# monahand1023/imageclust

Measured on AMD Instinct MI355X. Metric: images/sec (embed+Ward), higher is better.
Workload: dtype bf16; 1 GPU; the metric's size (configs[2]'s N=100000) on 1 GPU: 100000 synthetic 224x224x3 images (structured, seed 20250217; 100000 on this rank), ResNet50-v1 bf16 batch=256 -> 2048-d pooled E -> Ward min=5 max=50 (merge loop on GPU0) -> cluster ids on host; n_images_total=100000, embed_dim=2048, weights=synthetic seed 1, device=AMD Radeon Graphics (gfx950:sramecc+:xnack-)

## Files before the change

### imageclust_amd/csrc/ward.hip

```cpp
#pragma clang fp contract(off)

#include "icl_common.h"
#include "mfma_tile.h"
#include "ward_value.h"
typedef float f32x4 __attribute__((ext_vector_type(4)));

#include <algorithm>
#include <cmath>
#include <cstring>
#include <type_traits>

int icl_dist_mfma_launch(icl_ctx *ctx, const float *d_E, int64_t n, int d, float *d_out, const int64_t *d_rowoff, int64_t ld);
int icl_dist_center_launch(icl_ctx *ctx, const float *d_E, int64_t n, int d, int K, double *d_colsum, float *d_Ec, float *d_nrm, hipStream_t strm);
size_t icl_dist_colsum_doubles(int d);
int icl_dist_bound_launch(icl_ctx *ctx, const float *d_Ec, const float *d_nrm, const void *d_zero, int64_t n, int K, float ceps, float gam, float *d_out,
                          const int64_t *d_rowoff, int64_t tr_lo, int64_t tr_hi, hipStream_t strm);

bool icl_dist_i8_usable(int64_t n, int d);
size_t icl_dist_i8_pq_bytes(int64_t n, int d);
int icl_dist_bound_i8_launch(icl_ctx *ctx, const float *d_Ec, const float *d_nrm, int64_t n, int d, int K, float gam, void *d_pq, float *d_l1, int32_t *d_ex,
                             float *d_out, const int64_t *d_rowoff, hipStream_t strm, unsigned int *d_rowub);

typedef float f2 __attribute__((ext_vector_type(2)));

// ... 8 lines not shown
#define WB_R 128
#endif
#define WB_RL ((WB_R + 63) / 64)
#ifndef WB_NSP_LB
#define WB_NSP_LB 128
#endif
#define WB_NSP_X 64
#ifndef WB_SCAN_U
#define WB_SCAN_U 4
#endif
#ifndef WB_RM
#define WB_RM 2
#endif
__device__ __forceinline__ int wb_poll(const int32_t *p) { return __hip_atomic_load(p, __ATOMIC_RELAXED, __HIP_MEMORY_SCOPE_AGENT); }
__device__ __forceinline__ void wb_acquire() { __builtin_amdgcn_fence(__ATOMIC_ACQUIRE, "agent"); }
#define WB_NN_BOUND (-2)
#ifndef WB_LAZY_TOP
#define WB_LAZY_TOP 1
#endif
#define WB_PA_CAP 32
#define WB_WTOP 5
#define WB_PA_KEYS (WB_WTOP + 1)
__host__ __device__ __forceinline__ int wb_wtop(int nsp) { return nsp > 64 ? 3 : 5; }
#ifndef WB_LOOK
#define WB_LOOK 6
#endif
#ifndef WB_WPOP
#define WB_WPOP 4
#endif
#define WB_MAXWAVES (128 / (WB_WPOP + 1))
#define WB_ROLE_THREADS_OK(T) static_assert((T) % 64 == 0 && (T) / 64 <= WB_MAXWAVES && (T) / 64 <= 16, "spare / preselection roles: at most WB_MAXWAVES (and 16: sv / si / m3 scratch) waves per workgroup")
struct ward_batch_state {
    int32_t nb;
    int32_t a[WB_KMAX], b[WB_KMAX], sa[WB_KMAX], sb[WB_KMAX];
    float val[WB_KMAX];
    int32_t pre_n, pre_for_nb;
    int32_t pre_row[WB_KMAX], pre_nn[WB_KMAX], pre_sa[WB_KMAX], pre_sb[WB_KMAX];
    float pre_val[WB_KMAX];
    int32_t ov_n, ov_pad;
    int32_t ov_row[8], ov_nn[8];
    float ov_val[8];
    int32_t dirty_n, dirty_slot[2 * WB_K];
    int32_t epoch, spec_pad[2];
    int32_t spec_row[WB_R * WB_RM], spec_nn[WB_R * WB_RM], spec_done[WB_R];
    float spec_val[WB_R * WB_RM];
    int32_t commits, steps, slow, general;
    int32_t why[4];
    unsigned long long sum_live, sum_live_nb;
    unsigned long long sum_dep;
    unsigned long long ckey[WB_KMAX];
    unsigned long long ckey2[WB_KMAX];
#ifdef ICL_WARD_TIMERS
    unsigned long long dbg[8], dbg_t0, dbg2[3], dbg3[4], dbg4[4], dbg5[4], dbg6[8], dbg7[4];
    unsigned long long rf_stat[8];
#endif
    int32_t blk_next, blk_pad;
    int32_t pa_flag[WB_R], pa_cnt[WB_R];
    int32_t pa_rows[WB_R][WB_PA_CAP];
    unsigned long long pa_keys[WB_R][WB_PA_KEYS];
};

struct ward_state {
    int32_t done;
    int32_t t;
    int32_t cur_a, cur_b, cur_c;
    int32_t cur_valid;
    int32_t target;
    int32_t nlive;
    int32_t mv_from, mv_to;
    int32_t cur_sa, cur_sb;
    int32_t pre_row, pre_nn;
    float pre_val;
    int32_t foreign_flag;
    unsigned long long ckey;
// ... 813 lines not shown
    __syncthreads();
    float a = sv[0], b = v2[0], bw = w2[0];
    int ai = si[0], bi = i2[0];
    for (int w = 1; w < nw; ++w) {
        argmin_combine(a, ai, sv[w], si[w]);
        join(b, bi, bw, v2[w], i2[w], w2[w]);
    }
    v0 = a;
    i0 = ai;
    v1 = b;
    i1 = bi;
    w1 = bw;
    __syncthreads();
}

__device__ __forceinline__ void block_argmin_b3(float &v0, int &i0, float &b1, int &c1, float &b2, int &c2, float &b3, float *sv, int *si)
{
    auto cex = [](float &x, int &xc, float &y, int &yc) {
        const bool sw = y < x || (y == x && yc >= 0 && xc < 0);
        const float tx = sw ? y : x, ty = sw ? x : y;
        const int txc = sw ? yc : xc, tyc = sw ? xc : yc;
        x = tx; xc = txc; y = ty; yc = tyc;
    };
    auto join = [&](float &p1, int &q1, float &p2, int &q2, float &p3, float o1, int oc1, float o2, int oc2, float o3) {
        cex(p1, q1, o1, oc1);
        cex(p2, q2, o2, oc2);
        cex(p2, q2, o1, oc1);
        p3 = fminf(fminf(p3, o3), fminf(o1, o2));
    };
#pragma unroll
    for (int off = 32; off > 0; off >>= 1) {
        const float ov = __shfl_down(v0, off, 64);
        const int oi = __shfl_down(i0, off, 64);
        argmin_combine(v0, i0, ov, oi);
        const float o1 = __shfl_down(b1, off, 64), o2 = __shfl_down(b2, off, 64), o3 = __shfl_down(b3, off, 64);
        const int oc1 = __shfl_down(c1, off, 64), oc2 = __shfl_down(c2, off, 64);
        join(b1, c1, b2, c2, b3, o1, oc1, o2, oc2, o3);
    }
    __shared__ float j1[16], j2[16], j3[16];
    __shared__ int k1[16], k2[16];
    const int lane = threadIdx.x & 63, wid = threadIdx.x >> 6, nw = blockDim.x >> 6;
    if (lane == 0) {
        sv[wid] = v0;
// ... 8 lines not shown
    for (int w = 1; w < nw; ++w) {
        argmin_combine(a, ai, sv[w], si[w]);
        join(x1, y1, x2, y2, x3, j1[w], k1[w], j2[w], k2[w], j3[w]);
    }
    v0 = a; i0 = ai;
    b1 = x1; c1 = y1; b2 = x2; c2 = y2; b3 = x3;
    __syncthreads();
}

#ifdef ICL_WARD_TIMERS
__device__ unsigned long long g_walk_dbg[8];
__device__ unsigned long long g_main_dbg[12];
__device__ unsigned long long g_rs_dbg[8];
__device__ unsigned long long g_scan_dbg[8];
#endif
__device__ __forceinline__ void scan_row_min(float *__restrict__ row, int64_t len, const int32_t *__restrict__ msz, const int32_t *__restrict__ mcid,
                                             int my_id, int my_size, int max_size, const int *ex, int nex, float &bv, int &bi, float *sv, int *si,
                                             const wrefine &rf, float *scr, const uint32_t *__restrict__ mpk = nullptr)
{
    if (!(rf.E && (my_id < rf.n || rf.lb))) {
        WB_TIMER(const unsigned long long ts0 = wall_clock64();)
        scan_row_m(row, len, msz, mcid, my_id, my_size, max_size, ex, nex, bv, bi, mpk);
        WB_TIMER(const unsigned long long ts1 = wall_clock64();)
        block_argmin(bv, bi, sv, si);
        WB_TIMER(if (threadIdx.x == 0 && gridDim.x > 1) {
            atomicAdd(&g_scan_dbg[0], ts1 - ts0);
            atomicAdd(&g_scan_dbg[1], wall_clock64() - ts1);
            atomicAdd(&g_scan_dbg[2], 1ull);
            atomicAdd(&g_scan_dbg[3], (unsigned long long)len);
        })
        return;
    }
    auto excluded = [&](int c) { return wex_hit(ex, nex, c); };
    float tv = ICL_MAXF, lv = ICL_MAXF, lv2 = ICL_MAXF;
    int ti = -1, lc = -1;
    WB_TIMER(const unsigned long long tp0 = wall_clock64();)
    if (mpk) {
        const int szb = wpk_bits(max_size);
        const uint32_t smask = (1u << szb) - 1u;
        const uint32_t lim_u = max_size > my_size ? (uint32_t)(max_size - my_size) : 0u;
        const unsigned long long none = (unsigned long long)__float_as_uint(ICL_MAXF) << 32;
        unsigned long long tbest = none, l1 = none;
        uint32_t l2 = __float_as_uint(ICL_MAXF);
        const int64_t nvec = len >> 2;
        auto slow = [&](float v, uint32_t k, int col) {
            const int m = (int)(k & smask), c = (int)(k >> szb);
            if (!(m > 0 && m + my_size <= max_size && c < my_id)) return;
            const uint32_t vb = __float_as_uint(v);
            if (vb >> 31) {
                const uint32_t Lb = vb & 0x7fffffffu;
                const unsigned long long bk = ((unsigned long long)Lb << 32) | (unsigned)col;
                if (bk < l1) {
                    if (!excluded(c)) {
                        const uint32_t o = (uint32_t)(l1 >> 32);
                        l2 = o < l2 ? o : l2;
                        l1 = bk;
                    }
                } else
                    l2 = Lb < l2 ? Lb : l2;
// ... 57 lines not shown
                    slow(v[j].x, k[j].x, col);
                    slow(v[j].y, k[j].y, col + 1);
                    slow(v[j].z, k[j].z, col + 2);
                    slow(v[j].w, k[j].w, col + 3);
                }
            } else {
                const uint32_t h = (uint32_t)(g1 >> 32), o = (uint32_t)(l1 >> 32);
                if (g1 < l1) {
                    l2 = o < l2 ? o : l2;
                    l2 = g2 < l2 ? g2 : l2;
                    l1 = g1;
                } else
                    l2 = h < l2 ? h : l2;
            }
        };
        for (int64_t q0 = threadIdx.x; q0 < nvec; q0 += WB_SCAN_U * (int64_t)blockDim.x) {
            float4 v[WB_SCAN_U];
            uint4 k[WB_SCAN_U];
            load_group(q0, v, k);
            reduce_group(q0, v, k);
        }
        for (int64_t q = nvec * 4 + threadIdx.x; q < len; q += blockDim.x) slow(row[q], mpk[q], (int)q);
        if (tbest < none) {
            tv = __uint_as_float((uint32_t)(tbest >> 32));
            ti = (int)(unsigned)(tbest & 0xffffffffull);
        }
        if (l1 < none) {
            lv = __uint_as_float((uint32_t)(l1 >> 32));
            lc = (int)(unsigned)(l1 & 0xffffffffull);
        }
        lv2 = __uint_as_float(l2 < __float_as_uint(ICL_MAXF) ? l2 : __float_as_uint(ICL_MAXF));
    } else
    ward_row_visit(row, len, msz, mcid, [&](float v, int m, int c, int col) {
        if (!(m > 0 && m + my_size <= max_size && c < my_id)) return;
        if (wflagged(v)) {
            const float L = fabsf(v);
            if (L < lv) {
                if (!excluded(c)) {
                    lv2 = lv;
                    lv = L;
                    lc = col;
                }
            } else if (L < lv2)
                lv2 = L;
        } else if (v < tv || (v == tv && c < ti)) {
            if (!excluded(c)) {
                tv = v;
                ti = c;
            }
        }
    });
    WB_TIMER(const unsigned long long tp1 = wall_clock64();)
    int lc2 = -1;
    float lv3 = ICL_MAXF;
    block_argmin_b3(tv, ti, lv, lc, lv2, lc2, lv3, sv, si);
    WB_TIMER(const unsigned long long tp2 = wall_clock64();)
    WB_TIMER(if (threadIdx.x == 0 && gridDim.x > 1) {
        atomicAdd(&g_rs_dbg[0], 1ull);
        atomicAdd(&g_rs_dbg[1], tp1 - tp0);
        atomicAdd(&g_rs_dbg[2], tp2 - tp1);
        atomicAdd(&g_rs_dbg[4], (unsigned long long)len);
    })
    if (lc < 0 || lv > tv) {
        bv = tv;
        bi = ti;
        return;
    }
    if (rf.stat && threadIdx.x == 0) atomicAdd(&rf.stat[0], 1ull);
    if ((rf.d & 3) == 0 && rf.margin == 0.0f) {
        const int c = mcid[lc];
        const bool two = lc2 >= 0 && lv2 <= tv && blockDim.x >= 128;
        const int c2 = two ? mcid[lc2] : -1;
        if (threadIdx.x < (two ? 128 : 64)) {
            const int wv = (int)threadIdx.x >> 6;
            const int lcw = wv ? lc2 : lc, cw = wv ? c2 : c;
            const float *yc = wcent(rf, my_id);
            const float *xc = wcent(rf, cw);
// ... 141 lines not shown
        st->mv_from = st->mv_to = -1;
        st->pre_row = st->pre_nn = -1;
        st->pre_val = ICL_MAXF;
        st->ckey = ~0ull;
        st->B.nb = 0;
        st->B.pre_n = 0;
        st->B.pre_for_nb = -1;
        st->B.commits = st->B.steps = st->B.slow = st->B.general = 0;
        st->B.why[0] = st->B.why[1] = st->B.why[2] = st->B.why[3] = 0;
        st->B.sum_live = st->B.sum_live_nb = 0;
        st->B.sum_dep = 0;
        st->B.epoch = 1;
        st->B.dirty_n = 0;
        st->B.ov_n = 0;
        for (int j = 0; j < WB_R; ++j) st->B.spec_done[j] = st->B.pa_flag[j] = 0;
        for (int j = 0; j < WB_KMAX; ++j) st->B.ckey[j] = st->B.ckey2[j] = ~0ull;
        st->B.blk_next = 0;
#ifdef ICL_WARD_TIMERS
        for (int j = 0; j < 8; ++j) st->B.dbg[j] = 0;
        for (int j = 0; j < 3; ++j) st->B.dbg2[j] = 0;
        for (int j = 0; j < 4; ++j) st->B.dbg3[j] = st->B.dbg4[j] = 0;
        st->B.dbg4[3] = ~0ull;
        for (int j = 0; j < 4; ++j) st->B.dbg5[j] = 0;
        for (int j = 0; j < 8; ++j) st->B.dbg6[j] = 0;
        for (int j = 0; j < 4; ++j) st->B.dbg7[j] = 0;
        for (int j = 0; j < 8; ++j) st->B.rf_stat[j] = 0;
#endif
    }
}

// ... 434 lines not shown
        if (lane == 0) out[q] = m;
        if (kept && lane == q) *kept = m;
        if (m == ~0ull || (m & 1ull)) {
            ended = true;
            continue;
        }
        if (head == m) {
            ++stg;
            head = stg == 1 ? k2 : ((k2 == ~0ull || !has_rest) ? ~0ull : (k2 | 1ull));
        }
    }
    const unsigned long long rest = ended ? ~0ull : wave_min_u64(head);
    if (lane == 0) out[ntop] = rest == ~0ull ? rest : (rest | 1ull);
}

template <int K>
__device__ __forceinline__ void ward_spec_rescan(int nsp, int wg, int64_t n, const int32_t *__restrict__ asz, const float *__restrict__ rowmin,
                                 const int32_t *__restrict__ rownn, float *__restrict__ Dtri, const int64_t *__restrict__ rowoff,
                                 const int32_t *__restrict__ msz, const int32_t *__restrict__ mcid,
                                 int max_size, ward_state *__restrict__ st, float *sv, int *si, const wrefine &rf, const uint32_t *__restrict__ mpk = nullptr)
{
    __shared__ int excl[2 * K + WEX_WORDS];
    __shared__ int lcnt;
    __shared__ int lrows[WB_PA_CAP];
    __shared__ int mine[WB_RM];
    constexpr int WPOP = WB_LAZY_TOP ? WB_WPOP : WB_WTOP;
    __shared__ unsigned long long wstream[WB_MAXWAVES * (WB_WPOP + 1)];
    __shared__ unsigned long long mk[WB_LOOK + 1];
    static_assert(WPOP <= WB_WPOP && WB_LOOK >= WB_WTOP + 1 && WB_LOOK < 64, "the slice's merge holds two entries per lane");
    if (st->done) return;
    const int nb = st->B.nb, t0 = st->t, epoch = st->B.epoch;
    if (nb <= 0 || t0 + nb >= st->target) return;
    if (threadIdx.x < WEX_WORDS) excl[2 * K + threadIdx.x] = 0;
    if (threadIdx.x == 0) lcnt = 0;
    __syncthreads();
    if (threadIdx.x < 2 * K) {
        const int j = threadIdx.x >> 1;
        wex_add(excl, 2 * K, threadIdx.x, j < nb ? ((threadIdx.x & 1) ? st->B.b[j] : st->B.a[j]) : -1);
    }
    __syncthreads();
    const int lane = threadIdx.x & 63, wave = threadIdx.x >> 6, nwave = blockDim.x >> 6;
    WB_TIMER(const unsigned long long ta0 = wall_clock64();)
    const int64_t nvec = (n + t0 + 3) >> 2;
    const int64_t nchunk = (nvec + 3) >> 2;
    unsigned long long k1 = ~0ull, k2 = ~0ull;
    int nseen = 0;
    for (int64_t pp = threadIdx.x;; pp += blockDim.x) {
// ... 95 lines not shown
#pragma unroll
        for (int e = 0; e < WB_RL; ++e) {
            const int sl = lane + 64 * e;
            cnt_l[e] = (sl < nsp && have_all) ? __hip_atomic_load(&st->B.pa_cnt[sl], __ATOMIC_RELAXED, __HIP_MEMORY_SCOPE_AGENT) : 0;
            int inc = cnt_l[e];
#pragma unroll
            for (int off = 1; off < 64; off <<= 1) {
                const int o = __shfl_up(inc, off, 64);
                if (lane >= off) inc += o;
            }
            first[e] = base + inc - cnt_l[e];
            base += __shfl(inc, 63, 64);
        }
        const int total = base;
        if (wg == 0 && lane == 0) st->B.sum_dep += (unsigned long long)total;
        if (lane < WB_RM) mine[lane] = -1;
#pragma unroll
        for (int e = 0; e < WB_RL; ++e)
            for (int z = 0; z < cnt_l[e]; ++z) {
                const int idx = first[e] + z;
                if (idx >= wg && (idx - wg) % nsp == 0 && (idx - wg) / nsp < WB_RM)
                    mine[(idx - wg) / nsp] = __hip_atomic_load(&st->B.pa_rows[lane + 64 * e][z], __ATOMIC_RELAXED, __HIP_MEMORY_SCOPE_AGENT);
            }
    }
    __syncthreads();
    WB_TIMER(const unsigned long long tb0 = wall_clock64();)
    WB_TIMER(if (threadIdx.x == 0) atomicMax(&st->B.dbg6[0], tb0);)
    for (int m = 0; m < WB_RM; ++m) {
        const int r = mine[m];
        float rv = ICL_MAXF;
        int ri = -1;
        if (r >= 0) {
            WB_TIMER(const unsigned long long tr0 = wall_clock64();)
            scan_row_min(Dtri + rowoff[r], ward_row_len_rf(r, n, rf), msz, mcid, r, asz[r], max_size, excl, 2 * K, rv, ri, sv, si, rf, sv + 1024, mpk);
            WB_TIMER(if (threadIdx.x == 0) {
                const unsigned long long dt = wall_clock64() - tr0;
                atomicAdd(&st->B.dbg6[r < n ? 2 : 4], dt);
                atomicAdd(&st->B.dbg6[r < n ? 3 : 5], 1ull);
                atomicMax(&st->B.dbg6[6], dt);
                atomicMax(&st->B.dbg7[0], dt);
            })
        }
        if (threadIdx.x == 0) {
            st->B.spec_row[m * WB_R + wg] = r;
            st->B.spec_val[m * WB_R + wg] = rv;
            st->B.spec_nn[m * WB_R + wg] = ri;
        }
    }
    if (threadIdx.x == 0) {
        __hip_atomic_store(&st->B.spec_done[wg], epoch, __ATOMIC_RELEASE, __HIP_MEMORY_SCOPE_AGENT);
    }
}

template <int K>
__device__ __forceinline__ void ward_preselect_batch(int nsp, int64_t n, const int32_t *__restrict__ asz, float *__restrict__ rowmin, int32_t *__restrict__ rownn,
                                     float *__restrict__ Dtri, const int64_t *__restrict__ rowoff, const int32_t *__restrict__ msz,
                                     const int32_t *__restrict__ mcid, int max_size,
                                     ward_state *__restrict__ st, float *sv, int *si, int *sh, const wrefine &rf, const uint32_t *__restrict__ mpk = nullptr)
{
    __shared__ int excl[2 * K + WEX_WORDS];
    __shared__ unsigned long long wstream[16 * (WB_WTOP + 1)];
// ... 125 lines not shown
                            for (int spin = 0; spin < 20000 && !oke; ++spin) {
                                oke = wb_poll(&st->B.spec_done[sw]) == epoch;
                                if (!oke) __builtin_amdgcn_s_sleep(4);
                            }
                            ok &= oke;
                        }
                        wb_acquire();
                        spl_n = __all(ok) ? nsp : 0;
                        if (spl_n) {
#pragma unroll
                            for (int e = 0; e < WB_RL; ++e) {
                                const int sw = lane + 64 * e;
                                if (sw < nsp) {
#pragma unroll
                                    for (int m = 0; m < WB_RM; ++m) {
                                        spl_row[e * WB_RM + m] = __hip_atomic_load(&st->B.spec_row[m * WB_R + sw], __ATOMIC_RELAXED, __HIP_MEMORY_SCOPE_AGENT);
                                        spl_nn[e * WB_RM + m] = __hip_atomic_load(&st->B.spec_nn[m * WB_R + sw], __ATOMIC_RELAXED, __HIP_MEMORY_SCOPE_AGENT);
                                        spl_val[e * WB_RM + m] = __hip_atomic_load(&st->B.spec_val[m * WB_R + sw], __ATOMIC_RELAXED, __HIP_MEMORY_SCOPE_AGENT);
                                    }
                                }
                            }
                        }
                    }
                    unsigned long long hm = 0;
                    int sn = -1;
                    float sval = ICL_MAXF;
#pragma unroll
                    for (int m = 0; m < SPL; ++m) {
                        const unsigned long long h2 = __ballot(spl_n > 0 && spl_row[m] == r);
                        if (h2 && !hm) {
                            hm = h2;
// ... 771 lines not shown
#endif
__global__ __launch_bounds__(WL_THREADS) void ward_update_lb_kernel(int64_t S, const int32_t *__restrict__ slot_id, const int32_t *__restrict__ asz,
                                                                   const int64_t *__restrict__ rowoff, const int32_t *__restrict__ mcol,
                                                                   const int32_t *__restrict__ msz, const int32_t *__restrict__ mcid,
                                                                   float *__restrict__ Dtri, ward_state *__restrict__ st, int max_size, int64_t n,
                                                                   float *__restrict__ rowmin, int32_t *__restrict__ rownn, const wrefine rf,
                                                                   const uint32_t *__restrict__ mpk, int nsp)
{
    WB_ROLE_THREADS_OK(WL_THREADS);
    static_assert(WL_THREADS % WL_SLOTS == 0, "thread groups of WL_SLOTS lanes share the picks");
    __shared__ __attribute__((aligned(16))) float lds[1024 + (WL_THREADS / 64) * 256];
    float *sv = lds;
    int *si = reinterpret_cast<int *>(sv + 16);
    int *sh = si + 16;
    if (blockIdx.x < nsp) {
        ward_spec_rescan<WL_K>(nsp, (int)blockIdx.x, n, asz, rowmin, rownn, Dtri, rowoff, msz, mcid, max_size, st, sv, si, rf, mpk);
        WB_TIMER(if (threadIdx.x == 0) atomicMax(&st->B.dbg5[0], wall_clock64());)
        return;
    }
    if (blockIdx.x == nsp) {
        WB_TIMER(const unsigned long long t0 = wall_clock64();)
        WB_TIMER(if (threadIdx.x == 0) st->B.dbg_t0 = t0;)
        ward_preselect_batch<WL_K>(nsp, n, asz, rowmin, rownn, Dtri, rowoff, msz, mcid, max_size, st, sv, si, sh, rf, mpk);
        WB_TIMER(if (threadIdx.x == 0) st->B.dbg[0] += wall_clock64() - t0;)
        return;
    }
    const int lane = threadIdx.x & 63, wave = threadIdx.x >> 6;
    WB_TIMER(const unsigned long long tm0 = wall_clock64();)
    WB_TIMER(if (threadIdx.x == 0 && blockIdx.x > nsp + 1) atomicMin(&st->B.dbg4[3], tm0);)
    int pre_sx = 0;
    int64_t pre_rx = 0;
// ... 270 lines not shown
        st->B.dbg7[1] += st->B.dbg7[0];
        st->B.dbg7[0] = 0;
        st->B.dbg5[0] = 0;
        st->B.dbg3[3] = 0;
        st->B.dbg4[3] = ~0ull;
    })
    {
        constexpr int NW = (int)((offsetof(ward_state, B) + offsetof(ward_batch_state, pa_flag)) / 4);
        for (int q = threadIdx.x; q < NW; q += WB_FIN_THREADS) reinterpret_cast<int *>(&ls)[q] = reinterpret_cast<const int *>(st)[q];
        if (threadIdx.x == 0) {
            npk = 0;
        }
    }
    __syncthreads();
    if (ls.done) return;
    const int nbp = ls.B.nb, t0 = ls.t, nlive0 = ls.nlive, target = ls.target;
    const int lane = threadIdx.x & 63, wave = threadIdx.x >> 6;
    if (wave == 0) {
        int J = nbp;
        {
            float cm = ICL_MAXF;
            if (lane < nbp) {
                const unsigned long long k = ls.B.ckey[lane < WB_KMAX ? lane : 0];
                if (k != ~0ull) cm = __uint_as_float((unsigned)(k >> 32));
            }
            float pm = __shfl_up(cm, 1, 64);
            if (lane == 0) pm = ICL_MAXF;
#pragma unroll
            for (int off = 1; off < K; off <<= 1) {
                const float o = __shfl_up(pm, off, 64);
// ... 27 lines not shown
                mpk[cc] = ((uint32_t)c << wpk_bits(max_size)) | (uint32_t)(ls.B.sa[j] + ls.B.sb[j]);
                mpk[cb] = 0u;
            }
            rowmin[a] = ICL_MAXF;
            rowmin[b] = ICL_MAXF;
            rowmin[c] = key == ~0ull ? ICL_MAXF : __uint_as_float((unsigned)(key >> 32));
            rownn[c] = key == ~0ull ? -1 : WB_NN_BOUND;
        }
        if (full0 && lane < ls.B.ov_n) {
            rowmin[ls.B.ov_row[lane]] = ls.B.ov_val[lane];
            rownn[ls.B.ov_row[lane]] = ls.B.ov_nn[lane];
        }
#pragma unroll
        for (int e = 0; e < WB_RL; ++e) {
            const int sw = lane + 64 * e;
            if (J == nbp && J > 0 && sw < WB_R && ls.B.spec_done[sw] == ls.B.epoch) {
#pragma unroll
                for (int m = 0; m < WB_RM; ++m) {
                    const int sr = ls.B.spec_row[m * WB_R + sw];
                    if (sr >= 0) {
                        rowmin[sr] = ls.B.spec_val[m * WB_R + sw];
                        rownn[sr] = ls.B.spec_nn[m * WB_R + sw];
                    }
                }
            }
        }
        if (lane == 0 && J > 0) {
            st->nlive = nlive0 - J;
            st->t = t0 + J;
            st->B.steps = ls.B.steps + 1;
            st->B.commits = ls.B.commits + J;
        }
        const int t1 = t0 + J, pn0 = ls.B.pre_n;
        int np = 0;
// ... 321 lines not shown
                    mpk[cb] = 0u;
                }
            }
            rowmin[a] = ICL_MAXF;
            rowmin[b] = ICL_MAXF;
            rowmin[c] = key == ~0ull ? ICL_MAXF : __uint_as_float((unsigned)(key >> 32));
            rownn[c] = key == ~0ull ? -1 : rf.lb ? WB_NN_BOUND : (int)(key & 0xffffffffu);
        }
        if (full0 && lane < ls.B.ov_n) {
            rowmin[ls.B.ov_row[lane]] = ls.B.ov_val[lane];
            rownn[ls.B.ov_row[lane]] = ls.B.ov_nn[lane];
        }
#pragma unroll
        for (int e = 0; e < WB_RL; ++e) {
            const int sw = lane + 64 * e;
            if (J == nbp && sw < WB_R && ls.B.spec_done[sw] == ls.B.epoch) {
#pragma unroll
                for (int m = 0; m < WB_RM; ++m) {
                    const int sr = ls.B.spec_row[m * WB_R + sw];
                    if (sr >= 0) {
                        rowmin[sr] = ls.B.spec_val[m * WB_R + sw];
                        rownn[sr] = ls.B.spec_nn[m * WB_R + sw];
                    }
                }
            }
        }
        if (lane == 0) {
            st->nlive = nlive0 - J;
            st->t = t0 + J;
            st->B.steps = ls.B.steps + 1;
            st->B.commits = ls.B.commits + J;
        }
    }
    if (wave == 0) {
// ... 1189 lines not shown
            w->graph_ceps = rf.ceps;
            w->graph_ex = (const void *)rf.ex;
        }
        for (int64_t t = 0; t < T; t += GRAPH_STEPS) ICL_HIP(ctx, hipGraphLaunch(w->graph_exec, ctx->stream));
    }
    }
    ICL_HIP(ctx, hipGetLastError());
    ICL_HIP(ctx, hipEventRecord(e2, ctx->stream));

    ICL_HIP(ctx, hipMemcpyAsync(&hst, w->st, sizeof hst, hipMemcpyDeviceToHost, ctx->stream));
    ICL_HIP(ctx, hipStreamSynchronize(ctx->stream));
    if (!(hst.done || hst.t >= T))
        return icl_fail(ctx, ICL_ERR_HIP, "merge loop did not converge: %d of %lld merges after the step budget (engine bug, not a property of the input)",
                        hst.t, (long long)T);
    const int64_t nmerge = hst.t;
#ifdef ICL_WARD_TIMERS
    if (batched && getenv("ICL_WARD_STATS"))
        fprintf(stderr, "[icl] batched ward: merges %d steps %d commits %d single-pick steps %d general-path steps %d\n", hst.t, hst.B.steps, hst.B.commits,
                hst.B.slow, hst.B.general);
    if (batched && getenv("ICL_WARD_STATS") && rf.E)
        fprintf(stderr, "[icl] distance bounds in the merge loop: %llu scans of singleton rows, %llu collecting passes, %llu evaluation rounds, %llu entries evaluated\n",
                hst.B.rf_stat[0], hst.B.rf_stat[1], hst.B.rf_stat[2], hst.B.rf_stat[3]);
    if (batched && getenv("ICL_WARD_STATS"))
        fprintf(stderr, "[icl] rows of new clusters: %s\n", lw ? "Lance-Williams" : "exact values (vector ALUs)");
    if (batched && getenv("ICL_WARD_STATS") && rf.E)
        fprintf(stderr, "[icl] distance bounds, initial row minima: %llu rows, %llu evaluation rounds, %llu entries evaluated (%.2f %% of the pairs)\n",
                hst.B.rf_stat[4], hst.B.rf_stat[6], hst.B.rf_stat[7], 100.0 * (double)hst.B.rf_stat[7] / (0.5 * (double)n * (double)(n - 1)));
    if (batched && getenv("ICL_WARD_STATS"))
        fprintf(stderr, "[icl] non-express finishes: truncated %d, preselection stale/empty %d, new-row-first/forwarding %d; preselection re-minimised %d rows whose partner had died; %.1f rows per step depended on the batch\n", hst.B.why[0], hst.B.why[1], hst.B.why[2], hst.B.why[3], (double)hst.B.sum_dep / (hst.B.steps ? hst.B.steps : 1));
    if (batched && getenv("ICL_WARD_STATS"))
// ... 550 lines not shown
```

Measured before the change: 71580 images/sec.

## Split speculative row re-scans into balanced pieces shared across spare workgroups

The spare workgroups' speculative re-scan used to assign whole rows round-robin, so one long row could dominate the step. Rows are now prefix-summed by length and the total is cut into balanced ranges per workgroup. Each workgroup scans its piece, and the last finisher combines the partial top-3 results through global slots and finalizes the row minimum. Per-entry epoch tags replace the per-workgroup done flag. This adds cross-workgroup atomics and synchronization and raises the risk of ordering bugs.

```diff
diff --git a/imageclust_amd/csrc/ward.hip b/imageclust_amd/csrc/ward.hip
--- a/imageclust_amd/csrc/ward.hip
+++ b/imageclust_amd/csrc/ward.hip
@@ -2,6 +2,7 @@
 
 #include "icl_common.h"
 #include "mfma_tile.h"
+#include "ward_pieces.h"
 #include "ward_value.h"
 typedef float f32x4 __attribute__((ext_vector_type(4)));
 
@@ -46,6 +47,9 @@
 #endif
 __device__ __forceinline__ int wb_poll(const int32_t *p) { return __hip_atomic_load(p, __ATOMIC_RELAXED, __HIP_MEMORY_SCOPE_AGENT); }
 __device__ __forceinline__ void wb_acquire() { __builtin_amdgcn_fence(__ATOMIC_ACQUIRE, "agent"); }
+#ifndef WB_SHARE_RESCAN
+#define WB_SHARE_RESCAN 1
+#endif
 #define WB_NN_BOUND (-2)
 #ifndef WB_LAZY_TOP
 #define WB_LAZY_TOP 1
@@ -76,6 +80,7 @@
     int32_t epoch, spec_pad[2];
     int32_t spec_row[WB_R * WB_RM], spec_nn[WB_R * WB_RM], spec_done[WB_R];
     float spec_val[WB_R * WB_RM];
+    int32_t spec_ep[WB_R * WB_RM];
     int32_t commits, steps, slow, general;
     int32_t why[4];
     unsigned long long sum_live, sum_live_nb;
@@ -90,6 +95,9 @@
     int32_t pa_flag[WB_R], pa_cnt[WB_R];
     int32_t pa_rows[WB_R][WB_PA_CAP];
     unsigned long long pa_keys[WB_R][WB_PA_KEYS];
+    int32_t sp_tick[WB_R * WB_RM];
+    float sp_slot[WB_R][2][8];
+    unsigned long long sp_rows, sp_pieces;
 };
 
 struct ward_state {
@@ -933,19 +941,24 @@
     __syncthreads();
 }
 
+__device__ __forceinline__ void b3_cex(float &x, int &xc, float &y, int &yc)
+{
+    const bool sw = y < x || (y == x && yc >= 0 && xc < 0);
+    const float tx = sw ? y : x, ty = sw ? x : y;
+    const int txc = sw ? yc : xc, tyc = sw ? xc : yc;
+    x = tx; xc = txc; y = ty; yc = tyc;
+}
+__device__ __forceinline__ void b3_join(float &p1, int &q1, float &p2, int &q2, float &p3, float o1, int oc1, float o2, int oc2, float o3)
+{
+    b3_cex(p1, q1, o1, oc1);
+    b3_cex(p2, q2, o2, oc2);
+    b3_cex(p2, q2, o1, oc1);
+    p3 = fminf(fminf(p3, o3), fminf(o1, o2));
+}
 __device__ __forceinline__ void block_argmin_b3(float &v0, int &i0, float &b1, int &c1, float &b2, int &c2, float &b3, float *sv, int *si)
 {
-    auto cex = [](float &x, int &xc, float &y, int &yc) {
-        const bool sw = y < x || (y == x && yc >= 0 && xc < 0);
-        const float tx = sw ? y : x, ty = sw ? x : y;
-        const int txc = sw ? yc : xc, tyc = sw ? xc : yc;
-        x = tx; xc = txc; y = ty; yc = tyc;
-    };
     auto join = [&](float &p1, int &q1, float &p2, int &q2, float &p3, float o1, int oc1, float o2, int oc2, float o3) {
-        cex(p1, q1, o1, oc1);
-        cex(p2, q2, o2, oc2);
-        cex(p2, q2, o1, oc1);
-        p3 = fminf(fminf(p3, o3), fminf(o1, o2));
+        b3_join(p1, q1, p2, q2, p3, o1, oc1, o2, oc2, o3);
     };
 #pragma unroll
     for (int off = 32; off > 0; off >>= 1) {
@@ -984,35 +997,19 @@
 __device__ unsigned long long g_rs_dbg[8];
 __device__ unsigned long long g_scan_dbg[8];
 #endif
-__device__ __forceinline__ void scan_row_min(float *__restrict__ row, int64_t len, const int32_t *__restrict__ msz, const int32_t *__restrict__ mcid,
-                                             int my_id, int my_size, int max_size, const int *ex, int nex, float &bv, int &bi, float *sv, int *si,
-                                             const wrefine &rf, float *scr, const uint32_t *__restrict__ mpk = nullptr)
-{
-    if (!(rf.E && (my_id < rf.n || rf.lb))) {
-        WB_TIMER(const unsigned long long ts0 = wall_clock64();)
-        scan_row_m(row, len, msz, mcid, my_id, my_size, max_size, ex, nex, bv, bi, mpk);
-        WB_TIMER(const unsigned long long ts1 = wall_clock64();)
-        block_argmin(bv, bi, sv, si);
-        WB_TIMER(if (threadIdx.x == 0 && gridDim.x > 1) {
-            atomicAdd(&g_scan_dbg[0], ts1 - ts0);
-            atomicAdd(&g_scan_dbg[1], wall_clock64() - ts1);
-            atomicAdd(&g_scan_dbg[2], 1ull);
-            atomicAdd(&g_scan_dbg[3], (unsigned long long)len);
-        })
-        return;
-    }
+__device__ __forceinline__ void scan_row_pass_keyed(const float *__restrict__ row, int64_t c0, int64_t c1, int my_id, int my_size, int max_size, const int *ex,
+                                                    int nex, const wrefine &rf, const uint32_t *__restrict__ mpk, float &tv, int &ti, float &lv, int &lc,
+                                                    float &lv2)
+{
     auto excluded = [&](int c) { return wex_hit(ex, nex, c); };
-    float tv = ICL_MAXF, lv = ICL_MAXF, lv2 = ICL_MAXF;
-    int ti = -1, lc = -1;
-    WB_TIMER(const unsigned long long tp0 = wall_clock64();)
-    if (mpk) {
+    {
         const int szb = wpk_bits(max_size);
         const uint32_t smask = (1u << szb) - 1u;
         const uint32_t lim_u = max_size > my_size ? (uint32_t)(max_size - my_size) : 0u;
         const unsigned long long none = (unsigned long long)__float_as_uint(ICL_MAXF) << 32;
         unsigned long long tbest = none, l1 = none;
         uint32_t l2 = __float_as_uint(ICL_MAXF);
-        const int64_t nvec = len >> 2;
+        const int64_t nvec = c1 >> 2;
         auto slow = [&](float v, uint32_t k, int col) {
             const int m = (int)(k & smask), c = (int)(k >> szb);
             if (!(m > 0 && m + my_size <= max_size && c < my_id)) return;
@@ -1100,13 +1097,13 @@
                     l2 = h < l2 ? h : l2;
             }
         };
-        for (int64_t q0 = threadIdx.x; q0 < nvec; q0 += WB_SCAN_U * (int64_t)blockDim.x) {
+        for (int64_t q0 = (c0 >> 2) + threadIdx.x; q0 < nvec; q0 += WB_SCAN_U * (int64_t)blockDim.x) {
             float4 v[WB_SCAN_U];
             uint4 k[WB_SCAN_U];
             load_group(q0, v, k);
             reduce_group(q0, v, k);
         }
-        for (int64_t q = nvec * 4 + threadIdx.x; q < len; q += blockDim.x) slow(row[q], mpk[q], (int)q);
+        for (int64_t q = nvec * 4 + threadIdx.x; q < c1; q += blockDim.x) slow(row[q], mpk[q], (int)q);
         if (tbest < none) {
             tv = __uint_as_float((uint32_t)(tbest >> 32));
             ti = (int)(unsigned)(tbest & 0xffffffffull);
@@ -1116,7 +1113,38 @@
             lc = (int)(unsigned)(l1 & 0xffffffffull);
         }
         lv2 = __uint_as_float(l2 < __float_as_uint(ICL_MAXF) ? l2 : __float_as_uint(ICL_MAXF));
-    } else
+    }
+}
+
+__device__ __forceinline__ void scan_row_finish(float *__restrict__ row, int64_t len, const int32_t *__restrict__ msz, const int32_t *__restrict__ mcid,
+                                                int my_id, int my_size, int max_size, const int *ex, int nex, float &bv, int &bi, float *sv, int *si,
+                                                const wrefine &rf, float *scr, const uint32_t *__restrict__ mpk, float tv, int ti, float lv, int lc, float lv2,
+                                                int lc2, float lv3);
+
+__device__ __forceinline__ void scan_row_min(float *__restrict__ row, int64_t len, const int32_t *__restrict__ msz, const int32_t *__restrict__ mcid,
+                                             int my_id, int my_size, int max_size, const int *ex, int nex, float &bv, int &bi, float *sv, int *si,
+                                             const wrefine &rf, float *scr, const uint32_t *__restrict__ mpk = nullptr)
+{
+    if (!(rf.E && (my_id < rf.n || rf.lb))) {
+        WB_TIMER(const unsigned long long ts0 = wall_clock64();)
+        scan_row_m(row, len, msz, mcid, my_id, my_size, max_size, ex, nex, bv, bi, mpk);
+        WB_TIMER(const unsigned long long ts1 = wall_clock64();)
+        block_argmin(bv, bi, sv, si);
+        WB_TIMER(if (threadIdx.x == 0 && gridDim.x > 1) {
+            atomicAdd(&g_scan_dbg[0], ts1 - ts0);
+            atomicAdd(&g_scan_dbg[1], wall_clock64() - ts1);
+            atomicAdd(&g_scan_dbg[2], 1ull);
+            atomicAdd(&g_scan_dbg[3], (unsigned long long)len);
+        })
+        return;
+    }
+    auto excluded = [&](int c) { return wex_hit(ex, nex, c); };
+    float tv = ICL_MAXF, lv = ICL_MAXF, lv2 = ICL_MAXF;
+    int ti = -1, lc = -1;
+    WB_TIMER(const unsigned long long tp0 = wall_clock64();)
+    if (mpk)
+        scan_row_pass_keyed(row, 0, len, my_id, my_size, max_size, ex, nex, rf, mpk, tv, ti, lv, lc, lv2);
+    else
     ward_row_visit(row, len, msz, mcid, [&](float v, int m, int c, int col) {
         if (!(m > 0 && m + my_size <= max_size && c < my_id)) return;
         if (wflagged(v)) {
@@ -1147,6 +1175,15 @@
         atomicAdd(&g_rs_dbg[2], tp2 - tp1);
         atomicAdd(&g_rs_dbg[4], (unsigned long long)len);
     })
+    scan_row_finish(row, len, msz, mcid, my_id, my_size, max_size, ex, nex, bv, bi, sv, si, rf, scr, mpk, tv, ti, lv, lc, lv2, lc2, lv3);
+}
+
+__device__ __forceinline__ void scan_row_finish(float *__restrict__ row, int64_t len, const int32_t *__restrict__ msz, const int32_t *__restrict__ mcid,
+                                                int my_id, int my_size, int max_size, const int *ex, int nex, float &bv, int &bi, float *sv, int *si,
+                                                const wrefine &rf, float *scr, const uint32_t *__restrict__ mpk, float tv, int ti, float lv, int lc, float lv2,
+                                                int lc2, float lv3)
+{
+    WB_TIMER(const unsigned long long tp2 = wall_clock64();)
     if (lc < 0 || lv > tv) {
         bv = tv;
         bi = ti;
@@ -1318,6 +1355,8 @@
         st->B.dirty_n = 0;
         st->B.ov_n = 0;
         for (int j = 0; j < WB_R; ++j) st->B.spec_done[j] = st->B.pa_flag[j] = 0;
+        for (int j = 0; j < WB_R * WB_RM; ++j) st->B.spec_ep[j] = st->B.sp_tick[j] = 0;
+        st->B.sp_rows = st->B.sp_pieces = 0;
         for (int j = 0; j < WB_KMAX; ++j) st->B.ckey[j] = st->B.ckey2[j] = ~0ull;
         st->B.blk_next = 0;
 #ifdef ICL_WARD_TIMERS
@@ -1782,7 +1821,14 @@
     if (lane == 0) out[ntop] = rest == ~0ull ? rest : (rest | 1ull);
 }
 
-template <int K>
+template <bool SHARE> struct wsp_tables {};
+template <> struct wsp_tables<true> {
+    int64_t S[WB_R * WB_RM + 1], P[WB_R + 1];
+    int row[WB_R * WB_RM];
+    int rng[4], ji[4];
+    float jf[4];
+};
+template <int K, bool SHARE = false>
 __device__ __forceinline__ void ward_spec_rescan(int nsp, int wg, int64_t n, const int32_t *__restrict__ asz, const float *__restrict__ rowmin,
                                  const int32_t *__restrict__ rownn, float *__restrict__ Dtri, const int64_t *__restrict__ rowoff,
                                  const int32_t *__restrict__ msz, const int32_t *__restrict__ mcid,
@@ -1792,6 +1838,7 @@
     __shared__ int lcnt;
     __shared__ int lrows[WB_PA_CAP];
     __shared__ int mine[WB_RM];
+    __shared__ wsp_tables<SHARE> spt;
     constexpr int WPOP = WB_LAZY_TOP ? WB_WPOP : WB_WTOP;
     __shared__ unsigned long long wstream[WB_MAXWAVES * (WB_WPOP + 1)];
     __shared__ unsigned long long mk[WB_LOOK + 1];
@@ -1799,6 +1846,7 @@
     if (st->done) return;
     const int nb = st->B.nb, t0 = st->t, epoch = st->B.epoch;
     if (nb <= 0 || t0 + nb >= st->target) return;
+    const bool share = SHARE && mpk != nullptr && nsp == WB_NSP_LB;
     if (threadIdx.x < WEX_WORDS) excl[2 * K + threadIdx.x] = 0;
     if (threadIdx.x == 0) lcnt = 0;
     __syncthreads();
@@ -1924,18 +1972,192 @@
         }
         const int total = base;
         if (wg == 0 && lane == 0) st->B.sum_dep += (unsigned long long)total;
+        if constexpr (SHARE) {
+            if (share) {
+                constexpr int EPL = WB_RL * WB_RM;
+                const int nrow = total < nsp * WB_RM ? total : nsp * WB_RM;
+#pragma unroll
+                for (int e = 0; e < WB_RL; ++e)
+                    for (int z = 0; z < cnt_l[e]; ++z) {
+                        const int idx = first[e] + z;
+                        if (idx < nrow) {
+                            const int r = __hip_atomic_load(&st->B.pa_rows[lane + 64 * e][z], __ATOMIC_RELAXED, __HIP_MEMORY_SCOPE_AGENT);
+                            spt.row[idx] = r;
+                            spt.S[idx + 1] = ward_row_len_rf(r, n, rf);
+                        }
+                    }
+                if (lane == 0) spt.S[0] = 0;
+                auto wave_lds_sync = [] {
+                    __builtin_amdgcn_fence(__ATOMIC_RELEASE, "workgroup");
+                    __builtin_amdgcn_wave_barrier();
+                    __builtin_amdgcn_fence(__ATOMIC_ACQUIRE, "workgroup");
+                };
+                wave_lds_sync();
+                {
+                    int64_t loc[EPL], sum = 0;
+#pragma unroll
+                    for (int j = 0; j < EPL; ++j) {
+                        const int i = lane * EPL + j;
+                        sum += i < nrow ? spt.S[i + 1] : 0;
+                        loc[j] = sum;
+                    }
+                    int64_t inc = sum;
+#pragma unroll
+                    for (int off = 1; off < 64; off <<= 1) {
+                        const int64_t o = __shfl_up(inc, off, 64);
+                        if (lane >= off) inc += o;
+                    }
+#pragma unroll
+                    for (int j = 0; j < EPL; ++j) {
+                        const int i = lane * EPL + j;
+                        if (i < nrow) spt.S[i + 1] = inc - sum + loc[j];
+                    }
+                }
+                wave_lds_sync();
+                const int64_t minp = (int64_t)WB_SCAN_U * 4 * blockDim.x;
+#pragma unroll
+                for (int e = 0; e <= WB_RL; ++e) {
+                    const int k = lane + 64 * e;
+                    if (k <= nsp) spt.P[k] = wp_cut(spt.S, nrow, nsp, minp, k);
+                }
+                wave_lds_sync();
+                const int64_t p0 = spt.P[wg], p1 = spt.P[wg + 1];
+                int lo = 0x7fffffff, hi = -1;
+#pragma unroll
+                for (int j = 0; j < EPL; ++j) {
+                    const int i = lane * EPL + j;
+                    if (i < nrow && wp_holds(p0, p1, spt.S[i], spt.S[i + 1])) {
+                        lo = i < lo ? i : lo;
+                        hi = i > hi ? i : hi;
+                    }
+                }
+#pragma unroll
+                for (int off = 32; off > 0; off >>= 1) {
+                    const int a = __shfl_xor(lo, off, 64), b = __shfl_xor(hi, off, 64);
+                    lo = a < lo ? a : lo;
+                    hi = b > hi ? b : hi;
+                }
+                if (lane == 0) {
+                    spt.rng[0] = lo;
+                    spt.rng[1] = hi;
+                }
+            }
+        }
         if (lane < WB_RM) mine[lane] = -1;
-#pragma unroll
-        for (int e = 0; e < WB_RL; ++e)
-            for (int z = 0; z < cnt_l[e]; ++z) {
-                const int idx = first[e] + z;
-                if (idx >= wg && (idx - wg) % nsp == 0 && (idx - wg) / nsp < WB_RM)
-                    mine[(idx - wg) / nsp] = __hip_atomic_load(&st->B.pa_rows[lane + 64 * e][z], __ATOMIC_RELAXED, __HIP_MEMORY_SCOPE_AGENT);
-            }
+        if (!share) {
+#pragma unroll
+            for (int e = 0; e < WB_RL; ++e)
+                for (int z = 0; z < cnt_l[e]; ++z) {
+                    const int idx = first[e] + z;
+                    if (idx >= wg && (idx - wg) % nsp == 0 && (idx - wg) / nsp < WB_RM)
+                        mine[(idx - wg) / nsp] = __hip_atomic_load(&st->B.pa_rows[lane + 64 * e][z], __ATOMIC_RELAXED, __HIP_MEMORY_SCOPE_AGENT);
+                }
+        }
     }
     __syncthreads();
     WB_TIMER(const unsigned long long tb0 = wall_clock64();)
     WB_TIMER(if (threadIdx.x == 0) atomicMax(&st->B.dbg6[0], tb0);)
+    if constexpr (SHARE) {
+        if (share) {
+            const int i_lo = spt.rng[0], i_hi = spt.rng[1];
+            const int64_t p0 = spt.P[wg], p1 = spt.P[wg + 1];
+            for (int idx = i_lo; idx <= i_hi; ++idx) {
+                const int64_t s = spt.S[idx], e = spt.S[idx + 1], len = e - s;
+                const int64_t c0 = (p0 > s ? p0 : s) - s, c1 = (p1 < e ? p1 : e) - s;
+                if (c0 >= c1) continue;
+                WB_TIMER(const unsigned long long tr0 = wall_clock64();)
+                const int r = spt.row[idx], my_size = asz[r], entry = (idx / nsp) * WB_R + idx % nsp;
+                float *row = Dtri + rowoff[r];
+                float tv = ICL_MAXF, lv = ICL_MAXF, lv2 = ICL_MAXF, lv3 = ICL_MAXF;
+                int ti = -1, lc = -1, lc2 = -1;
+                scan_row_pass_keyed(row, c0, c1, r, my_size, max_size, excl, 2 * K, rf, mpk, tv, ti, lv, lc, lv2);
+                block_argmin_b3(tv, ti, lv, lc, lv2, lc2, lv3, sv, si);
+                bool fin = true;
+                if (c0 > 0 || c1 < len) {
+                    if (wave == 0) {
+                        bool hold[WB_RL];
+                        int np = 0, fw = nsp;
+#pragma unroll
+                        for (int q = 0; q < WB_RL; ++q) {
+                            const int w = lane + 64 * q;
+                            hold[q] = w < nsp && wp_holds(spt.P[w < nsp ? w : 0], spt.P[w < nsp ? w + 1 : 0], s, e);
+                            const unsigned long long hm = __ballot(hold[q]);
+                            np += __popcll(hm);
+                            if (hm && fw == nsp) fw = 64 * q + __ffsll((long long)hm) - 1;
+                        }
+                        int last = 0;
+                        if (lane == 0) {
+                            int32_t *sl = reinterpret_cast<int32_t *>(&st->B.sp_slot[wg][c0 > 0 ? 0 : 1][0]);
+                            const int32_t w7[7] = {(int32_t)__float_as_uint(tv), ti, (int32_t)__float_as_uint(lv), lc, (int32_t)__float_as_uint(lv2), lc2, (int32_t)__float_as_uint(lv3)};
+#pragma unroll
+                            for (int q = 0; q < 7; ++q) __hip_atomic_store(sl + q, w7[q], __ATOMIC_RELAXED, __HIP_MEMORY_SCOPE_AGENT);
+                            __builtin_amdgcn_fence(__ATOMIC_RELEASE, "agent");
+                            asm volatile("s_waitcnt vmcnt(0)" ::: "memory");
+                            last = __hip_atomic_fetch_add(&st->B.sp_tick[entry], 1, __ATOMIC_RELAXED, __HIP_MEMORY_SCOPE_AGENT) == np - 1;
+                        }
+                        last = __shfl(last, 0, 64);
+                        if (last) {
+                            wb_acquire();
+                            float jv = ICL_MAXF, j1 = ICL_MAXF, j2 = ICL_MAXF, j3 = ICL_MAXF;
+                            int ji = -1, k1 = -1, k2 = -1;
+#pragma unroll
+                            for (int q = 0; q < WB_RL; ++q) {
+                                if (!hold[q]) continue;
+                                const int w = lane + 64 * q;
+                                const int32_t *sl = reinterpret_cast<const int32_t *>(&st->B.sp_slot[w][w == fw ? 1 : 0][0]);
+                                int32_t w7[7];
+#pragma unroll
+                                for (int z = 0; z < 7; ++z) w7[z] = __hip_atomic_load(sl + z, __ATOMIC_RELAXED, __HIP_MEMORY_SCOPE_AGENT);
+                                argmin_combine(jv, ji, __uint_as_float((uint32_t)w7[0]), w7[1]);
+                                b3_join(j1, k1, j2, k2, j3, __uint_as_float((uint32_t)w7[2]), w7[3], __uint_as_float((uint32_t)w7[4]), w7[5], __uint_as_float((uint32_t)w7[6]));
+                            }
+#pragma unroll
+                            for (int off = 32; off > 0; off >>= 1) {
+                                const float ov = __shfl_down(jv, off, 64), o1 = __shfl_down(j1, off, 64), o2 = __shfl_down(j2, off, 64), o3 = __shfl_down(j3, off, 64);
+                                const int oi = __shfl_down(ji, off, 64), oc1 = __shfl_down(k1, off, 64), oc2 = __shfl_down(k2, off, 64);
+                                argmin_combine(jv, ji, ov, oi);
+                                b3_join(j1, k1, j2, k2, j3, o1, oc1, o2, oc2, o3);
+                            }
+                            if (lane == 0) {
+                                spt.jf[0] = jv; spt.jf[1] = j1; spt.jf[2] = j2; spt.jf[3] = j3;
+                                spt.ji[0] = ji; spt.ji[1] = k1; spt.ji[2] = k2;
+                                atomicAdd(&st->B.sp_rows, 1ull);
+                                atomicAdd(&st->B.sp_pieces, (unsigned long long)np);
+                            }
+                        }
+                        if (lane == 0) spt.rng[2] = last;
+                    }
+                    __syncthreads();
+                    fin = spt.rng[2] != 0;
+                    if (fin) {
+                        tv = spt.jf[0]; lv = spt.jf[1]; lv2 = spt.jf[2]; lv3 = spt.jf[3];
+                        ti = spt.ji[0]; lc = spt.ji[1]; lc2 = spt.ji[2];
+                    }
+                    __syncthreads();
+                }
+                if (fin) {
+                    float rv = ICL_MAXF;
+                    int ri = -1;
+                    scan_row_finish(row, len, msz, mcid, r, my_size, max_size, excl, 2 * K, rv, ri, sv, si, rf, sv + 1024, mpk, tv, ti, lv, lc, lv2, lc2, lv3);
+                    if (threadIdx.x == 0) {
+                        st->B.spec_row[entry] = r;
+                        st->B.spec_val[entry] = rv;
+                        st->B.spec_nn[entry] = ri;
+                        st->B.spec_ep[entry] = epoch;
+                    }
+                }
+                WB_TIMER(if (threadIdx.x == 0) {
+                    const unsigned long long dt = wall_clock64() - tr0;
+                    atomicAdd(&st->B.dbg6[r < n ? 2 : 4], dt);
+                    atomicAdd(&st->B.dbg6[r < n ? 3 : 5], 1ull);
+                    atomicMax(&st->B.dbg6[6], dt);
+                    atomicMax(&st->B.dbg7[0], dt);
+                })
+            }
+            if (threadIdx.x == 0) __hip_atomic_store(&st->B.spec_done[wg], epoch, __ATOMIC_RELEASE, __HIP_MEMORY_SCOPE_AGENT);
+            return;
+        }
+    }
     for (int m = 0; m < WB_RM; ++m) {
         const int r = mine[m];
         float rv = ICL_MAXF;
@@ -1955,6 +2177,7 @@
             st->B.spec_row[m * WB_R + wg] = r;
             st->B.spec_val[m * WB_R + wg] = rv;
             st->B.spec_nn[m * WB_R + wg] = ri;
+            st->B.spec_ep[m * WB_R + wg] = epoch;
         }
     }
     if (threadIdx.x == 0) {
@@ -2110,7 +2333,8 @@
                                 if (sw < nsp) {
 #pragma unroll
                                     for (int m = 0; m < WB_RM; ++m) {
-                                        spl_row[e * WB_RM + m] = __hip_atomic_load(&st->B.spec_row[m * WB_R + sw], __ATOMIC_RELAXED, __HIP_MEMORY_SCOPE_AGENT);
+                                        const bool cur = __hip_atomic_load(&st->B.spec_ep[m * WB_R + sw], __ATOMIC_RELAXED, __HIP_MEMORY_SCOPE_AGENT) == epoch;
+                                        spl_row[e * WB_RM + m] = cur ? __hip_atomic_load(&st->B.spec_row[m * WB_R + sw], __ATOMIC_RELAXED, __HIP_MEMORY_SCOPE_AGENT) : -1;
                                         spl_nn[e * WB_RM + m] = __hip_atomic_load(&st->B.spec_nn[m * WB_R + sw], __ATOMIC_RELAXED, __HIP_MEMORY_SCOPE_AGENT);
                                         spl_val[e * WB_RM + m] = __hip_atomic_load(&st->B.spec_val[m * WB_R + sw], __ATOMIC_RELAXED, __HIP_MEMORY_SCOPE_AGENT);
                                     }
@@ -2912,7 +3136,7 @@
     int *si = reinterpret_cast<int *>(sv + 16);
     int *sh = si + 16;
     if (blockIdx.x < nsp) {
-        ward_spec_rescan<WL_K>(nsp, (int)blockIdx.x, n, asz, rowmin, rownn, Dtri, rowoff, msz, mcid, max_size, st, sv, si, rf, mpk);
+        ward_spec_rescan<WL_K, WB_SHARE_RESCAN != 0>(nsp, (int)blockIdx.x, n, asz, rowmin, rownn, Dtri, rowoff, msz, mcid, max_size, st, sv, si, rf, mpk);
         WB_TIMER(if (threadIdx.x == 0) atomicMax(&st->B.dbg5[0], wall_clock64());)
         return;
     }
@@ -3213,6 +3437,7 @@
     }
     __syncthreads();
     if (ls.done) return;
+    for (int q = threadIdx.x; q < WB_R * WB_RM; q += WB_FIN_THREADS) st->B.sp_tick[q] = 0;
     const int nbp = ls.B.nb, t0 = ls.t, nlive0 = ls.nlive, target = ls.target;
     const int lane = threadIdx.x & 63, wave = threadIdx.x >> 6;
     if (wave == 0) {
@@ -3270,10 +3495,10 @@
 #pragma unroll
         for (int e = 0; e < WB_RL; ++e) {
             const int sw = lane + 64 * e;
-            if (J == nbp && J > 0 && sw < WB_R && ls.B.spec_done[sw] == ls.B.epoch) {
+            if (J == nbp && J > 0 && sw < WB_R) {
 #pragma unroll
                 for (int m = 0; m < WB_RM; ++m) {
-                    const int sr = ls.B.spec_row[m * WB_R + sw];
+                    const int sr = ls.B.spec_ep[m * WB_R + sw] == ls.B.epoch ? ls.B.spec_row[m * WB_R + sw] : -1;
                     if (sr >= 0) {
                         rowmin[sr] = ls.B.spec_val[m * WB_R + sw];
                         rownn[sr] = ls.B.spec_nn[m * WB_R + sw];
@@ -3625,10 +3850,10 @@
 #pragma unroll
         for (int e = 0; e < WB_RL; ++e) {
             const int sw = lane + 64 * e;
-            if (J == nbp && sw < WB_R && ls.B.spec_done[sw] == ls.B.epoch) {
+            if (J == nbp && sw < WB_R) {
 #pragma unroll
                 for (int m = 0; m < WB_RM; ++m) {
-                    const int sr = ls.B.spec_row[m * WB_R + sw];
+                    const int sr = ls.B.spec_ep[m * WB_R + sw] == ls.B.epoch ? ls.B.spec_row[m * WB_R + sw] : -1;
                     if (sr >= 0) {
                         rowmin[sr] = ls.B.spec_val[m * WB_R + sw];
                         rownn[sr] = ls.B.spec_nn[m * WB_R + sw];
@@ -4848,6 +5073,8 @@
         return icl_fail(ctx, ICL_ERR_HIP, "merge loop did not converge: %d of %lld merges after the step budget (engine bug, not a property of the input)",
                         hst.t, (long long)T);
     const int64_t nmerge = hst.t;
+    if (batched && lbm && getenv("ICL_WARD_STATS"))
+        fprintf(stderr, "[icl] shared re-scans: %llu rows completed from %llu pieces\n", hst.B.sp_rows, hst.B.sp_pieces);
 #ifdef ICL_WARD_TIMERS
     if (batched && getenv("ICL_WARD_STATS"))
         fprintf(stderr, "[icl] batched ward: merges %d steps %d commits %d single-pick steps %d general-path steps %d\n", hst.t, hst.B.steps, hst.B.commits,
diff --git a/imageclust_amd/csrc/ward_pieces.h b/imageclust_amd/csrc/ward_pieces.h
--- /dev/null
+++ b/imageclust_amd/csrc/ward_pieces.h
@@ -0,0 +1,66 @@
+#pragma once
+#include <stdint.h>
+
+#if defined(__HIPCC__) || defined(__CUDACC__)
+#define WP_HD __host__ __device__ __forceinline__
+#else
+#define WP_HD static inline
+#endif
+
+WP_HD int64_t wp_cut(const int64_t *S, int total, int nsp, int64_t minp, int k)
+{
+    const int64_t T = S[total];
+    if (k <= 0) return 0;
+    if (k >= nsp) return T;
+    const int64_t g = ((int64_t)k * T + nsp - 1) / nsp;
+    if (g >= T) return T;
+    int lo = 0, hi = total - 1;
+    while (lo < hi) {
+        const int mid = (lo + hi + 1) >> 1;
+        if (S[mid] <= g)
+            lo = mid;
+        else
+            hi = mid - 1;
+    }
+    const int64_t s = S[lo], len = S[lo + 1] - s, c = g - s;
+    if (c == 0) return g;
+    const int64_t grid = (T / nsp >= 2 * minp) ? 4 : minp;
+    int64_t cc = (c + grid - 1) / grid * grid;
+    if (cc < minp) cc = minp;
+    if (len - cc < minp) cc = len;
+    return s + cc;
+}
+
+WP_HD bool wp_holds(int64_t p0, int64_t p1, int64_t s, int64_t e) { return (p0 > s ? p0 : s) < (p1 < e ? p1 : e); }
+
+WP_HD int wp_pieces_of(const int64_t *S, int total, int nsp, int64_t minp, int w, int32_t *row, int64_t *c0, int64_t *c1, int cap)
+{
+    const int64_t p0 = wp_cut(S, total, nsp, minp, w), p1 = wp_cut(S, total, nsp, minp, w + 1);
+    int np = 0;
+    for (int i = 0; i < total; ++i) {
+        if (!wp_holds(p0, p1, S[i], S[i + 1])) continue;
+        if (np < cap) {
+            row[np] = i;
+            c0[np] = (p0 > S[i] ? p0 : S[i]) - S[i];
+            c1[np] = (p1 < S[i + 1] ? p1 : S[i + 1]) - S[i];
+        }
+        ++np;
+    }
+    return np;
+}
+
+WP_HD int wp_row_pieces(const int64_t *S, int total, int nsp, int64_t minp, int i, int *first_wg)
+{
+    int cnt = 0, first = -1;
+    int64_t p0 = 0;
+    for (int w = 0; w < nsp; ++w) {
+        const int64_t p1 = wp_cut(S, total, nsp, minp, w + 1);
+        if (wp_holds(p0, p1, S[i], S[i + 1])) {
+            if (first < 0) first = w;
+            ++cnt;
+        }
+        p0 = p1;
+    }
+    if (first_wg) *first_wg = first;
+    return cnt;
+}
```

Result: slower. 69230 images/sec (-3.3%).
